# bottledspace/refraction-raytracing-dxr

Hardware: AMD Instinct MI355X
Metric: Mrays/s (primary+refracted) at 1920x1080, monkey.obj (higher is better)
Workload: dtype f32

## Files before the change

refraction_raytracing_dxr_amd/_build.py:

```python
import os
import shutil
import subprocess

PKG = os.path.dirname(os.path.abspath(__file__))
CSRC = os.path.join(PKG, "csrc")
LIB = os.path.join(PKG, "librrdxr.so")
DEMO = os.path.join(PKG, "rrdemo")

DEVICE_SOURCES = ["rr_bvh_build.hip", "rr_render_fused.hip", "rr_render_paths.hip", "rr_render_lds.hip", "rr_render_stream.hip",
                  "rr_query.hip", "rr_query_multi.hip", "rr_frame.hip", "rr_shade_rays.hip", "rr_render_samples.hip",
                  "rr_render_adaptive.hip", "rr_render_lens.hip", "rr_render_spectral.hip", "rr_render_materials.hip"]
HOST_SOURCES = ["rr_capi.cpp", "rr_capi_build.cpp", "rr_capi_dispatch.cpp", "rr_capi_orbit.cpp", "rr_capi_query.cpp", "rr_capi_comm.cpp",
                "rr_choice.cpp", "host/rr_host_camera.cpp", "host/rr_host_mesh.cpp", "host/rr_host_image.cpp", "host/rr_host_partition.cpp",
                "host/Mesh.cpp", "host/RefractionDemo.cpp"]
HEADERS = ["rr_types.h", "rr_context.h", "rr_choice.h", "rr_device.h", "rr_launch.h", "rr_render_common.h", "rr_render_materials.h", "host/Mesh.hpp", "host/RefractionDemo.hpp", "host/rr_host_lens.h",
           "../../include/rrdxr.h"]

COMMON = ["-O3", "-std=c++17", "-fPIC", "-ffp-contract=off", "-fno-fast-math", "-Wall", "-Wno-unused-function"]
DEVICE_FLAGS = ["--offload-arch=gfx950", "-fno-gpu-rdc"] + os.environ.get("RR_EXTRA_DEFINES", "").split()


def _hipcc():
    exe = shutil.which("hipcc") or "/opt/rocm/bin/hipcc"
    if not os.path.exists(exe):
        raise RuntimeError("hipcc not found: the HIP extension cannot be built")
    return exe


def _stale(target, deps):
    if not os.path.exists(target):
        return True
    t = os.path.getmtime(target)
    return any((not os.path.exists(d)) or os.path.getmtime(d) > t for d in deps)


def build(force=False, verbose=False):
    hipcc = _hipcc()
    srcs = [os.path.join(CSRC, s) for s in DEVICE_SOURCES + HOST_SOURCES]
    deps = srcs + [os.path.join(CSRC, h) for h in HEADERS] + [os.path.abspath(__file__)]
    objdir = os.path.join(PKG, "build")
    os.makedirs(objdir, exist_ok=True)
    stamp = os.path.join(objdir, "flags.txt")
# ... 30 lines not shown
```

refraction_raytracing_dxr_amd/csrc/rr_capi.cpp:

```cpp
#include "rr_context.h"

#include <dlfcn.h>
#include <new>

static_assert(CHOICE_TILE == (uint32_t)TILE && CHOICE_STREAM_MAX_GEN == STREAM_MAX_GEN, "rr_choice.h mirrors rr_types.h");

static_assert(sizeof(rr_vertex) == 32, "Vertex stride (Mesh.cpp:45)");
static_assert(sizeof(rr_instance_desc) == 64, "D3D12_RAYTRACING_INSTANCE_DESC");
static_assert(sizeof(rr_scene_constants) == 80, "SceneConstants");
static_assert(sizeof(rr_ray) == sizeof(rr_ray_dev) && sizeof(rr_hit) == sizeof(rr_hit_dev), "ray/hit ABI");
static_assert(offsetof(rr_ray, instance_mask) == 36 && offsetof(rr_ray_dev, instance_mask) == 36, "rr_ray.instance_mask");

namespace {
struct Roctx {
    int (*push)(const char*) = nullptr;
    int (*pop)() = nullptr;
    Roctx()
    {
        for (const char* lib : { "librocprofiler-sdk-roctx.so", "libroctx64.so" }) {
            if (void* h = dlopen(lib, RTLD_LAZY | RTLD_LOCAL)) {
                push = reinterpret_cast<int (*)(const char*)>(dlsym(h, "roctxRangePushA"));
                pop = reinterpret_cast<int (*)()>(dlsym(h, "roctxRangePop"));
                if (push && pop) return;
                push = nullptr; pop = nullptr;
// ... 117 lines not shown
    rr_context* ctx = new (std::nothrow) rr_context();
    if (!ctx) return RR_ERR_OUT_OF_MEMORY;
    ctx->device = device_ordinal;
    ctx->n_cus = prop.multiProcessorCount > 0 ? prop.multiProcessorCount : 256;
    if (hipSetDevice(device_ordinal) != hipSuccess || ctx->own_stream.create(hipStreamNonBlocking) != hipSuccess ||
        ctx->d_cnt.alloc(1) != hipSuccess || ctx->d_tickets.alloc((rr_context::MAX_LANES + 1) * LDS_TICKET_WORDS) != hipSuccess) {
        delete ctx;
        return RR_ERR_DEVICE;
    }
    ctx->stream = ctx->own_stream.get();
    (void)hipMemsetAsync(ctx->d_cnt.get(), 0, sizeof(CounterBlock), ctx->stream);
    (void)hipMemsetAsync(ctx->d_tickets.get(), 0, (rr_context::MAX_LANES + 1) * LDS_TICKET_WORDS * sizeof(uint32_t), ctx->stream);
    if (const char* e = getenv("RR_DEBUG_KERNEL"))
        ctx->dbg.kernel = !strcmp(e, "fused") ? 1 : !strcmp(e, "lds") ? 4 : !strcmp(e, "paths") ? 5 : !strcmp(e, "stream") ? 10 : 0;
    if (const char* e = getenv("RR_DEBUG_STACK")) ctx->dbg.stack = atoi(e);
    if (const char* e = getenv("RR_DEBUG_TICKET")) ctx->dbg_ticket_blocks = atoi(e);
    if (const char* e = getenv("RR_DEBUG_SHAPE")) ctx->dbg_shape = atoi(e);
    if (const char* e = getenv("RR_DEBUG_REFINE_GROUPS")) ctx->dbg_refine_groups = std::max(atoi(e), 0);
    if (const char* e = getenv("RR_DEBUG_TLAS32")) ctx->dbg.tlas32 = atoi(e) != 0;
    if (const char* e = getenv("RR_DEBUG_TILE_ORDER")) ctx->dbg_tile_order = atoi(e) != 0;
    if (const char* e = getenv("RR_DEBUG_ASYNC")) { unsigned l = 2, sh = 2; if (sscanf(e, "%u,%u", &l, &sh) == 2 && l >= 1 && sh >= 1) { ctx->dbg_async[0] = l; ctx->dbg_async[1] = sh; ctx->dbg_async_set = true; } }
    if (const char* e = getenv("RR_DEBUG_DIAG")) ctx->dbg_diag = e;
    if (const char* e = getenv("RR_DEBUG_GROUP_TRACE")) ctx->dbg_group_trace = atoi(e) != 0;
    *out = ctx;
    return RR_OK;
}

int rr_destroy(rr_context* ctx)
{
    if (!ctx) return RR_ERR_INVALID_ARGUMENT;
    (void)hipSetDevice(ctx->device);
    (void)hipStreamSynchronize(ctx->stream);
    for (const Stream& s : ctx->lane_stream) if (s.get()) (void)hipStreamSynchronize(s.get());
    delete ctx;
    return RR_OK;
}

const char* rr_last_error(const rr_context* ctx) { return ctx ? ctx->err.c_str() : "null context"; }

int rr_set_stream(rr_context* ctx, void* hip_stream)
{
    if (int r = use_device(ctx)) return r;
    RR_HIP(hipStreamSynchronize(ctx->stream));
    ctx->stream = (hipStream_t)hip_stream;
    return RR_OK;
}

int rr_reset_stream(rr_context* ctx)
{
    if (int r = use_device(ctx)) return r;
    RR_HIP(hipStreamSynchronize(ctx->stream));
    ctx->stream = ctx->own_stream.get();
    return RR_OK;
}

int rr_wait(rr_context* ctx)
{
    if (int r = use_device(ctx)) return r;
    if (int r = join_lanes(ctx)) return r;
    RR_HIP(hipStreamSynchronize(ctx->stream));
    return RR_OK;
}

int rr_set_frames_in_flight(rr_context* ctx, uint32_t n)
{
    if (int r = use_device(ctx)) return r;
// ... 223 lines not shown
```

refraction_raytracing_dxr_amd/csrc/rr_capi_dispatch.cpp:

```cpp
#include "rr_context.h"

namespace {
int ensure_cams(rr_context* ctx, size_t n)
{
    return n <= ctx->d_cams.size() ? RR_OK : ctx->d_cams.grow(ctx, n < 64 ? 64 : n);
}

constexpr size_t STREAM_BUDGET_MAX = (size_t)48 << 30, STREAM_BUDGET_MIN = (size_t)1 << 30;
constexpr uint32_t STREAM_BLK = 1024;

size_t stream_budget(rr_context* ctx)
{
    if (ctx->strm_budget == 0) {
        size_t free_b = 0, total_b = 0;
        size_t b = STREAM_BUDGET_MAX;
        if (hipMemGetInfo(&free_b, &total_b) == hipSuccess) b = std::min(b, free_b / 6u);
        if (const char* e = getenv("RR_DEBUG_STREAM_BUDGET_GB")) { const long g = atol(e); if (g > 0 && g <= 200) b = (size_t)g << 30; }
        ctx->strm_budget = std::max(b, STREAM_BUDGET_MIN);
    }
    return ctx->strm_budget;
}

uint32_t lds_node_bytes(const MeshRes& m) { return m.n_nodes() * (uint32_t)sizeof(QNode); }

// ... 172 lines not shown
struct Launch {
    SceneDev sc;
    DispatchDev a;
    uint32_t need;
    const rr_scene_constants* h_cams; const rr_dispatch_params* p;
    FusedVariant fused;
};

int ensure_lds_park(rr_context* ctx, uint32_t slot, int max_reflect)
{
    const size_t park_need = (size_t)ctx->n_cus * 32 * (max_reflect <= 2 ? 2u : 8u) * 8 * 64;
    return ctx->d_park[slot].size() < park_need ? ctx->d_park[slot].grow(ctx, park_need) : RR_OK;
}

int launch_lds(rr_context* ctx, const Launch& L, bool stats)
{
    const MeshRes& m0 = ctx->meshes[(size_t)ctx->inst_host[0].blas];
    LdsDispatch q;
    memset(&q, 0, sizeof q);
    const uint32_t slot = stream_slot(ctx);
    q.tickets = ctx->d_tickets.get() + (size_t)slot * LDS_TICKET_WORDS;
    q.park_slots = L.p->max_reflect <= 2 ? 2u : 8u;
    if (int r = ensure_lds_park(ctx, slot, L.p->max_reflect)) return r;
    q.park = ctx->d_park[slot].get();
    uint32_t rect[4];
    (void)rr_host_screen_rect(m0.bounds, ((ctx->dbg_ticket_blocks & 3) == 1 || (L.p->flags & RR_DISPATCH_DEBUG_NO_CULL)) ? nullptr : L.h_cams, L.a.n_frames,
                     L.a.W, L.a.H, rect);
    if ((ctx->dbg_ticket_blocks & 3) == 2) rect[2] = rect[0];
    q.n_queues = (ctx->dbg_ticket_blocks & 64) ? 64u : (ctx->dbg_ticket_blocks & 128) ? LDS_QUEUES : 8u;
    q.home_xcc = (ctx->dbg_ticket_blocks & 16) ? 0u : 1u;
    q.rx0 = rect[0]; q.ry0 = rect[1]; q.rx1 = rect[2]; q.ry1 = rect[3];
    q.node_bytes = lds_node_bytes(m0);
    q.stack_entries = L.need + 1;
    RR_HIP(launch_render_lds(L.sc, L.a, q, ctx->n_cus, stats, ctx->stream, ctx->dbg_shape));
    return RR_OK;
}

int launch_kernel(rr_context* ctx, const Launch& L, int kernel, bool stats)
{
    if (kernel == K_STREAM) return render_stream(ctx, L.sc, L.a, L.a.n_frames, (int)L.need, stats);
    if (kernel == K_LDS) return launch_lds(ctx, L, stats);
    if (kernel == K_PATHS) RR_HIP(launch_render_paths(L.sc, L.a, (int)L.need, stats, ctx->stream));
    else RR_HIP(launch_render_fused(L.sc, L.a, L.fused.stack, L.fused.pend, stats, ctx->stream, L.fused.stack16));
    return RR_OK;
}

int time_candidates(rr_context* ctx, Launch L, int cand_a, int cand_b, float ms[2])
{
    if (cand_b == K_STREAM) if (int r = ensure_stream_buffers(ctx, stream_plan(ctx, L.a, L.a.n_frames))) return r;
    if (cand_a == K_LDS || cand_b == K_LDS) if (int r = ensure_lds_park(ctx, stream_slot(ctx), L.p->max_reflect)) return r;
    for (Event& e : ctx->ch_ev) if (!e.get()) RR_HIP(e.create(hipEventDefault));
    if (!ctx->d_cnt_trial.get()) RR_HIP(ctx->d_cnt_trial.alloc(1));
    RR_HIP(hipDeviceSynchronize());
    RR_HIP(hipMemsetAsync(ctx->d_cnt_trial.get(), 0, sizeof(CounterBlock), ctx->stream));
    point_counters(L.a, ctx->d_cnt_trial.get());
    if (int r = launch_kernel(ctx, L, cand_a, false)) return r;
    for (int c = 0; c < 2; ++c) {
        RR_HIP(hipEventRecord(ctx->ch_ev[2 * c].get(), ctx->stream));
        if (int r = launch_kernel(ctx, L, c == 0 ? cand_a : cand_b, false)) return r;
        RR_HIP(hipEventRecord(ctx->ch_ev[2 * c + 1].get(), ctx->stream));
    }
    RR_HIP(hipEventSynchronize(ctx->ch_ev[3].get()));
    RR_HIP(hipEventElapsedTime(&ms[0], ctx->ch_ev[0].get(), ctx->ch_ev[1].get()));
    RR_HIP(hipEventElapsedTime(&ms[1], ctx->ch_ev[2].get(), ctx->ch_ev[3].get()));
    return RR_OK;
}

// ... 213 lines not shown
```

refraction_raytracing_dxr_amd/csrc/rr_context.h:

```cpp
#pragma once
#include "../../include/rrdxr.h"

#include <hip/hip_runtime.h>

#include <algorithm>
#include <cmath>
#include <cstdio>
#include <cstdlib>
#include <cstring>
#include <string>
#include <vector>

#include "rr_choice.h"
#include "rr_launch.h"

namespace rr {

struct Range {
    explicit Range(const char* name);
    ~Range();
};

template <class T, bool Pinned = false> class Buf {
public:
// ... 121 lines not shown
    bool cam_set = false;
    DevBuf<CamDev> d_cams;
    static constexpr int CAM_SLOTS = 4;
    HostBuf<CamDev> h_cams[CAM_SLOTS];
    Event      h_cams_ev[CAM_SLOTS];
    bool       h_cams_busy[CAM_SLOTS] = {};
    uint32_t   h_cams_next = 0;

    uint32_t tile_rank = 0, tile_world = 1;

    static constexpr uint32_t MAX_LANES = 4;
    Stream      lane_stream[MAX_LANES];
    Event       lane_fork[MAX_LANES], lane_done[MAX_LANES];
    DevBuf<CamDev> lane_cams[MAX_LANES];
    bool        lane_busy[MAX_LANES] = {};
    uint32_t    frames_in_flight = 2;
    size_t      frame_base = 0;

    uint32_t W = 0, H = 0, frame_world = 0, frame_depth = 1;
    DevBuf<uint32_t> d_rgba8;
    DevBuf<float4>   d_f32;
    DevBuf<uint32_t> d_assembled;
    bool      have_f32 = false, have_frame = false, have_assembled = false;
    uint64_t  last_pixels = 0;
    uint64_t  accum_pixels = 0;
    bool      last_stats = false;

    DevBuf<CounterBlock> d_cnt;
    DevBuf<CounterBlock> d_cnt_trial;
    DevBuf<uint32_t> d_park[MAX_LANES + 1];
    char       last_kernel_name[96] = "";
    uint32_t   last_kernel = 0;
    DevBuf<uint32_t> d_tickets;

    DebugFacts dbg = { 0, 0, false };
    int  dbg_ticket_blocks = 0;
    bool dbg_group_trace = true;
    bool dbg_async_set = false;
    uint32_t dbg_async[2] = { 2, 2 };
    bool dbg_tile_order = true;
    int  dbg_shape = 0;
    int  dbg_refine_groups = 0;
    std::string dbg_diag;

    Event ev_begin, ev_end;
    std::vector<Event> kev;
    uint32_t kev_used = 0;

    StreamSet strm[MAX_LANES + 1];
    size_t    strm_budget = 0;
    ChoiceClass ch[3];
    Event      ch_ev[4];

    DevBuf<rr_ray_dev> d_rays;
    DevBuf<rr_hit_dev> d_hits;
    DevBuf<uint32_t>   d_counts;
    DevBuf<float4>     d_out_f32;
    DevBuf<uint32_t>   d_out_rgba8, d_out_n;
    DevBuf<uint32_t>   d_adaptive_taken;
    DevBuf<float4>     d_adaptive_ws;
    DevBuf<MatDev>     d_mats;
    uint32_t n_mats = 0, max_material = 0;
};

namespace rr {

// ... 53 lines not shown
```

refraction_raytracing_dxr_amd/csrc/rr_launch.h:

```cpp
#pragma once
#include <hip/hip_runtime.h>
#include "rr_types.h"
#include "host/rr_host_lens.h"

namespace rr {

struct alignas(16) rr_ray_dev { float origin[3]; float tmin; float dir[3]; float tmax; uint32_t flags; uint32_t instance_mask; uint32_t pad[2]; };
struct rr_hit_dev { float t, u, v; uint32_t prim, inst, hit; };
static_assert(sizeof(rr_ray_dev) == 48 && sizeof(rr_hit_dev) == 24, "ABI layout");

hipError_t launch_render_fused(const SceneDev& sc, const DispatchDev& a, int stack, int pend, bool stats, hipStream_t s,
                               bool stack16 = false);
const char* last_render_kernel_name();
void set_render_kernel_name(const char* fmt, ...) __attribute__((format(printf, 1, 2)));
hipError_t launch_render_paths(const SceneDev& sc, const DispatchDev& a, int stack, bool stats, hipStream_t s);
int lds_kernel_shape(uint32_t node_bytes, uint32_t stack_entries, size_t* lds_bytes, int min_shape = 0);
hipError_t launch_render_lds(const SceneDev& sc, const DispatchDev& a, LdsDispatch q, int n_cus, bool stats, hipStream_t s, int min_shape = 0);
hipError_t launch_render_stream(const SceneDev& sc, const DispatchDev& a, const StreamDev& s, int stack, uint32_t n_wg, bool stats, hipStream_t st);
hipError_t launch_env_lookup(const SceneDev& sc, const float* dirs, uint32_t n, float* rgb, hipStream_t s);
hipError_t launch_trace_rays(const SceneDev& sc, const rr_ray_dev* rays, uint32_t n, rr_hit_dev* hits, uint32_t* err,
                             int stack, hipStream_t s);
hipError_t launch_query_rays(const SceneDev& sc, const rr_ray_dev* rays, uint32_t n, rr_hit_dev* hits, uint32_t inst0_mask, int stack,
                             hipStream_t s);
constexpr uint32_t RR_QUERY_MULTI_MAX_K = 16;
hipError_t launch_query_multi(const SceneDev& sc, const rr_ray_dev* rays, uint32_t n, uint32_t k, rr_hit_dev* hits, uint32_t* counts,
                              uint32_t inst0_mask, int stack, hipStream_t s);
hipError_t launch_shade_rays(const SceneDev& sc, const DispatchDev& a, const rr_ray_dev* rays, uint32_t n, float4* f32, uint32_t* rgba8,
                             uint32_t* n_rays, int stack, int pend, bool stack16, hipStream_t s);
struct SampleOffsets { static constexpr uint32_t MAX = 64; float v[2 * MAX]; };
hipError_t launch_render_samples(const SceneDev& sc, const DispatchDev& a, const CamDev& cam, const SampleOffsets& off, uint32_t n_samples,
                                 float4* f32, uint32_t* rgba8, uint32_t* n_rays, int stack, int pend, bool stack16, hipStream_t s);
hipError_t launch_render_lens(const SceneDev& sc, const DispatchDev& a, const CamDev& cam, const SampleOffsets& off, const SampleOffsets& loff,
                              const LensDev& lens, uint32_t n_samples, float4* f32, uint32_t* rgba8, uint32_t* n_rays, int stack, int pend,
                              bool stack16, hipStream_t s);
struct BandTable { static constexpr uint32_t MAX = SampleOffsets::MAX; float ior[MAX]; float inv_ior[MAX]; float weight[MAX][3]; };
hipError_t launch_render_spectral(const SceneDev& sc, const DispatchDev& a, const CamDev& cam, const SampleOffsets& off, const BandTable& bands,
                                  uint32_t n_samples, float4* f32, uint32_t* rgba8, uint32_t* n_rays, int stack, int pend, bool stack16,
                                  hipStream_t s);
hipError_t launch_shade_rays_mat(const SceneDev& sc, const DispatchDev& a, const MatDev* mats, uint32_t mat0, const rr_ray_dev* rays, uint32_t n,
                                 float4* f32, uint32_t* rgba8, uint32_t* n_rays, int stack, int pend, bool stack16, hipStream_t s);
hipError_t launch_render_materials(const SceneDev& sc, const DispatchDev& a, const CamDev& cam, const SampleOffsets& off, const MatDev* mats,
                                   uint32_t mat0, uint32_t n_samples, float4* f32, uint32_t* rgba8, uint32_t* n_rays, int stack, int pend,
                                   bool stack16, hipStream_t s);
struct AdaptiveWorkspace {
    float4* rec; uint32_t* cnt; uint32_t* list; unsigned long long* masks; uint32_t* base; uint32_t* total;
    uint64_t bytes;
    AdaptiveWorkspace(void* p, uint32_t W, uint32_t H)
    {
        const uint64_t n = (uint64_t)W * H, nb = (uint64_t)((W + 7u) / 8u) * ((H + 7u) / 8u);
        const uint64_t o_cnt = 16u * n, o_list = o_cnt + 4u * n, o_masks = (o_list + 4u * n + 15u) & ~(uint64_t)15u, o_base = o_masks + 8u * nb;
// ... 57 lines not shown
```

refraction_raytracing_dxr_amd/csrc/rr_render_common.h:

```cpp
#pragma once
#include <hip/hip_runtime.h>
#include <type_traits>
#include "rr_device.h"
#include "rr_launch.h"

#ifndef RR_FUSED_WAVES_PER_SIMD
#define RR_FUSED_WAVES_PER_SIMD(STACK) ((STACK) <= 19 ? 8 : (STACK) <= 22 ? 7 : (STACK) <= 26 ? 6 : (STACK) <= 31 ? 5 : (STACK) <= 39 ? 4 : 2)
#endif
#ifndef RR_TLAS_WAVES_PER_SIMD
#define RR_TLAS_WAVES_PER_SIMD(STACK) ((STACK) <= 31 ? 5 : (STACK) <= 39 ? 4 : 2)
#endif

namespace rr {


struct PendRay {
    float ox, oy, oz, dx, dy, dz, w;
    uint32_t meta;
};

__device__ __forceinline__ uint32_t compact1by1(uint32_t v)
{
    v &= 0x55555555u;
    v = (v ^ (v >> 1)) & 0x33333333u;
// ... 230 lines not shown
        p3[0] = (uint8_t)packed; p3[1] = (uint8_t)(packed >> 8); p3[2] = (uint8_t)(packed >> 16);
    } else {
        out_rgba8[o] = packed;
    }
    if (out_f32) out_f32[o] = make_float4(acc.x, acc.y, acc.z, 1.0f);
}

template <bool STATS>
__device__ __forceinline__ void flush_stats(const DispatchDev& a, const LaneStats& st, uint32_t shard, uint32_t lane)
{
    uint32_t wr = wave_reduce_add(st.rays);
    if (lane == 0 && wr) atomicAdd(&a.ray_shards[shard & (RAY_SHARDS - 1)], wr);
    if (STATS) {
        uint32_t v;
        v = wave_reduce_add(st.hits);  if (lane == 0 && v) atomicAdd(&a.counters[C_HITS], (unsigned long long)v);
        v = wave_reduce_add(st.miss);  if (lane == 0 && v) atomicAdd(&a.counters[C_MISSES], (unsigned long long)v);
        v = wave_reduce_add(st.term);  if (lane == 0 && v) atomicAdd(&a.counters[C_TERMINAL], (unsigned long long)v);
        v = wave_reduce_add(st.tir);   if (lane == 0 && v) atomicAdd(&a.counters[C_TIR], (unsigned long long)v);
        v = wave_reduce_add(st.cnt.nodes); if (lane == 0 && v) atomicAdd(&a.counters[C_NODES], (unsigned long long)v);
        v = wave_reduce_add(st.cnt.tris);  if (lane == 0 && v) atomicAdd(&a.counters[C_TRIS], (unsigned long long)v);
        v = wave_reduce_add(st.pixels); if (lane == 0 && v) atomicAdd(&a.counters[C_PRIMARY], (unsigned long long)v);
        v = wave_reduce_add(st.cnt.node_trips); if (lane == 0 && v) atomicAdd(&a.counters[C_NODE_TRIPS], (unsigned long long)v);
        v = wave_reduce_add(st.cnt.leaf_trips); if (lane == 0 && v) atomicAdd(&a.counters[C_LEAF_TRIPS], (unsigned long long)v);
        v = wave_reduce_add(st.passes); if (lane == 0 && v) atomicAdd(&a.counters[C_PASSES], (unsigned long long)v);
        if (lane == 0 && st.blocks) atomicAdd(&a.counters[C_WAVES], (unsigned long long)st.blocks);
        if (lane == 0 && st.bg_blocks) atomicAdd(&a.counters[C_BG_WAVES], (unsigned long long)st.bg_blocks);
        if (lane == 0 && (st.blocks || st.rays)) {
            atomicAdd(&a.counters[C_CLK_TICKS], (unsigned long long)(__builtin_amdgcn_s_memtime() - st.clk0));
            atomicAdd(&a.counters[C_CLK_REAL], (unsigned long long)(__builtin_amdgcn_s_memrealtime() - st.rt0));
        }
    }
}

__device__ __forceinline__ uint32_t tile_in_launch_order(const DispatchDev& a, uint32_t i, uint32_t limit)
{
    if (a.rt_w == 0u || i >= limit) return i;
    const uint32_t n_rect = a.rt_w * a.rt_h;
    if (i < n_rect) {
        const uint32_t row = a.rt_w == 1u ? i : __umulhi(i, a.rt_div_w);
        return (a.rt_y0 + row) * a.tiles_x + a.rt_x0 + (i - row * a.rt_w);
    }
    uint32_t j = i - n_rect;
    const uint32_t above = a.rt_y0 * a.tiles_x;
    if (j < above) return j;
    j -= above;
    const uint32_t per_row = a.tiles_x - a.rt_w, beside = per_row * a.rt_h;
    if (j < beside) {
        const uint32_t row = per_row == 1u ? j : __umulhi(j, a.rt_div_o), c = j - row * per_row;
        return (a.rt_y0 + row) * a.tiles_x + (c < a.rt_x0 ? c : c + a.rt_w);
    }
    return (a.rt_y0 + a.rt_h) * a.tiles_x + (j - beside);
}

struct BlockPos { uint32_t frame, tile_local, x0, y0, px0, py0; bool tile_ok, bg; };
__device__ __forceinline__ BlockPos wave_block_pos(const DispatchDev& a, uint32_t wb)
{
    BlockPos p;
    const uint32_t blk = wb >> 2, wave = wb & 3u;
    p.frame = blk % a.n_frames;
    uint32_t strip;
    block_to_tile(blk / a.n_frames, p.tile_local, strip);
    p.tile_ok = p.tile_local < a.n_local_tiles;
    p.bg = false;
    uint32_t tile;
    if (a.mesh_part) {
        const uint32_t k = p.tile_local;
// ... 16 lines not shown
```

refraction_raytracing_dxr_amd/csrc/rr_render_lds.hip:

```cpp
#include <hip/hip_runtime.h>
#include "rr_render_common.h"

namespace rr {

__device__ __forceinline__ BlockPos lds_tile_block(const DispatchDev& a, const LdsDispatch& q, uint32_t u, uint32_t j)
{
    BlockPos p;
    const uint32_t tile = a.n_frames == 1u ? u : __umulhi(u, q.div_frames);
    p.frame = u - tile * a.n_frames;
    p.tile_local = tile;
    p.tile_ok = tile < a.n_local_tiles;
    p.bg = false;
    const uint32_t ty = a.tiles_x == 1u ? tile : __umulhi(tile, q.div_tiles_x), tx = tile - ty * a.tiles_x;
    p.px0 = (j & 3u) * 8u; p.py0 = (j >> 2) * 8u;
    p.x0 = tx * TILE + p.px0; p.y0 = ty * TILE + p.py0;
    return p;
}

__device__ __forceinline__ BlockPos lds_rect_block(const DispatchDev& a, const LdsDispatch& q, uint32_t u, uint32_t j)
{
    BlockPos p;
    const uint32_t strip = a.n_frames == 1u ? u : __umulhi(u, q.div_frames), per_row = q.rect_bw >> 2;
    p.frame = u - strip * a.n_frames;
    const uint32_t row = per_row == 1u ? strip : __umulhi(strip, q.div_per_row), col = strip - row * per_row;
// ... 132 lines not shown
        if (w_arrived + 1u == (uint32_t)NW) {
            const uint32_t arrived = atomicAdd(&q.tickets[2u * LDS_QUEUES * 16u], 1u);
            if (arrived + 1u == gridDim.x) {
                for (uint32_t k = 0; k <= 2u * LDS_QUEUES; ++k) atomicExch(&q.tickets[k * 16u], 0u);
            }
        }
    }
}

constexpr struct { int nw, wgs; } LDS_SHAPES[] = { { 12, 2 }, { 16, 2 }, { 16, 1 } };
static size_t lds_shape_bytes(int i, uint32_t node_bytes, uint32_t stack_entries) { return (size_t)node_bytes + (size_t)LDS_SHAPES[i].nw * stack_entries * 64 * sizeof(uint16_t); }

int lds_kernel_shape(uint32_t node_bytes, uint32_t stack_entries, size_t* lds_bytes, int min_shape)
{
    for (int i = min_shape < 0 ? 0 : min_shape; i < 3; ++i) {
        const size_t need = lds_shape_bytes(i, node_bytes, stack_entries);
        if (need <= (size_t)(160 * 1024) / LDS_SHAPES[i].wgs - 512) { if (lds_bytes) *lds_bytes = need; return i; }
        if (min_shape <= 0) break;
    }
    return -1;
}

template <int SHAPE, bool STATS, bool DIAG = false>
static hipError_t launch_lds_nw(const SceneDev& sc, const DispatchDev& a, const LdsDispatch& q, int n_cus, hipStream_t s)
{
    constexpr int NW = LDS_SHAPES[SHAPE].nw, WGS = LDS_SHAPES[SHAPE].wgs;
    static const hipError_t attr = hipFuncSetAttribute(reinterpret_cast<const void*>(&k_render_lds<NW, WGS, STATS, DIAG>), hipFuncAttributeMaxDynamicSharedMemorySize, 159 * 1024);
    if (attr != hipSuccess) return attr;
    if (!DIAG) set_render_kernel_name("k_render_lds<%d, %d, %s, false>", NW, WGS, STATS ? "true" : "false");
    hipLaunchKernelGGL((k_render_lds<NW, WGS, STATS, DIAG>), dim3((uint32_t)n_cus * WGS), dim3(NW * 64), lds_shape_bytes(SHAPE, q.node_bytes, q.stack_entries), s, sc, a, q);
    return hipGetLastError();
}

hipError_t launch_render_lds(const SceneDev& sc, const DispatchDev& a, LdsDispatch q, int n_cus, bool stats, hipStream_t s, int min_shape)
{
    if (a.n_blocks == 0) return hipSuccess;
    const int shape = lds_kernel_shape(q.node_bytes, q.stack_entries, nullptr, min_shape);
    if (shape < 0) return hipErrorInvalidValue;
    {
        const uint32_t grid = (uint32_t)n_cus * (uint32_t)LDS_SHAPES[shape].wgs;
        if (q.n_queues > grid) q.n_queues = grid;
        if (q.n_queues > LDS_QUEUES) q.n_queues = LDS_QUEUES;
        if (q.n_queues < 1u) q.n_queues = 1u;
    }
    q.p2_tickets = a.n_local_tiles * a.n_frames;
    if (q.rx1 > q.rx0 && q.ry1 > q.ry0) {
        q.rx0 &= ~31u;
        q.rx1 = (q.rx1 + 31u) & ~31u;
    }
    const bool rect = q.rx1 > q.rx0 && q.ry1 > q.ry0;
    q.rect_bw = rect ? (q.rx1 - q.rx0) / 8u : 0u;
    q.p1_tickets = !rect ? 0u : (q.rect_bw / 4u) * ((q.ry1 - q.ry0) / 8u) * a.n_frames;
    if ((uint64_t)q.p2_tickets * a.n_frames >= 0xffffffffull || (uint64_t)q.p1_tickets * a.n_frames >= 0xffffffffull) return hipErrorInvalidValue;
    q.div_frames = (uint32_t)(0x100000000ull / a.n_frames) + 1u;
    q.div_tiles_x = (uint32_t)(0x100000000ull / a.tiles_x) + 1u;
    q.div_per_row = rect ? (uint32_t)(0x100000000ull / (q.rect_bw / 4u)) + 1u : 0u;
    static_assert(sizeof LDS_SHAPES / sizeof LDS_SHAPES[0] == 3, "lds_kernel_shape and the rungs below");
    if (a.diag) return launch_lds_nw<0, false, true>(sc, a, q, n_cus, s);
    if (shape == 0) return stats ? launch_lds_nw<0, true>(sc, a, q, n_cus, s) : launch_lds_nw<0, false>(sc, a, q, n_cus, s);
    if (shape == 1) return stats ? launch_lds_nw<1, true>(sc, a, q, n_cus, s) : launch_lds_nw<1, false>(sc, a, q, n_cus, s);
    return stats ? launch_lds_nw<2, true>(sc, a, q, n_cus, s) : launch_lds_nw<2, false>(sc, a, q, n_cus, s);
}

}
```

refraction_raytracing_dxr_amd/csrc/rr_render_stream.hip:

```cpp
#include <hip/hip_runtime.h>
#include "rr_render_common.h"

#ifndef RR_STREAM_WPS
#define RR_STREAM_WPS 6
#endif

namespace rr {

constexpr uint32_t SQ_BLK = 1024;
constexpr uint32_t SQ_NONE = 0xffffffffu;
constexpr uint32_t SQ_DEAD = 0xfffffffeu;
constexpr int TRAV_FIN = (int)0x80000001;
constexpr int TRAV_IDLE = (int)0x80000002;
constexpr uint8_t PIX_BLACK = 0, PIX_ONE_LEAF = 1, PIX_LEAVES = 2;

__device__ __forceinline__ void sq_finalize(const StreamDev& s, uint32_t qsel, uint32_t base, uint32_t used, uint32_t lane)
{
    if (lane < SQ_BLK / 64u) {
        const uint32_t lo = lane * 64u;
        s.fill[qsel][(base >> 6) + lane] = used > lo ? (used - lo < 64u ? used - lo : 64u) : 0u;
    }
}

__device__ __forceinline__ void sq_push(const StreamDev& s, uint32_t gen_out, uint32_t& base, uint32_t& used, bool have, f3 O, f3 D,
// ... 336 lines not shown
                    const uint32_t rank = __builtin_amdgcn_mbcnt_hi((uint32_t)(need >> 32), __builtin_amdgcn_mbcnt_lo((uint32_t)need, 0u));
                    if (node == TRAV_IDLE && rank < left) {
                        const uint32_t r = chunk * 64u + off + rank;
                        const uint32_t m = __float_as_uint(qin[(size_t)r * 3 + 2].x);
                        const float4 q0 = qin[(size_t)r * 3], q1 = qin[(size_t)r * 3 + 1];
                        rid = r;
                        start_ray(mk3(q0.x, q0.y, q0.z), mk3(q1.x, q1.y, q1.z), (m & META_INSIDE) != 0u, true);
                    }
                    const uint32_t asked = (uint32_t)__popcll(need);
                    off += asked < left ? asked : left;
                    need = __ballot(node == TRAV_IDLE);
                }
            }
        }
    }
    if (MODE != 2 && ob != SQ_NONE && ob != SQ_DEAD) sq_finalize(s, (gen + 1u) & 1u, ob, ou, lane);
    flush_stats<STATS>(a, st, blockIdx.x * 4u + wave, lane);
}

template <bool STATS>
__global__ __launch_bounds__(256) void k_stream_background(SceneDev sc, DispatchDev a, StreamDev s)
{
    const uint32_t wave = __builtin_amdgcn_readfirstlane(threadIdx.x >> 6), lane = threadIdx.x & 63u;
    const uint32_t wb = s.n_rect_wb + blockIdx.x * 4u + wave;
    LaneStats st;
    stats_clock_begin<STATS>(st);
    if (wb < a.n_blocks * 4u) {
        const BlockPos bp = wave_block_pos(a, wb);
        const uint32_t lx = compact1by1(lane), ly = compact1by1(lane >> 1);
        const uint32_t x = bp.x0 + lx, y = bp.y0 + ly;
        st.blocks = bp.tile_ok ? 1u : 0u;
        if (STATS) st.bg_blocks = st.blocks;
        if (bp.tile_ok && x < a.W && y < a.H) {
            const CamDev& cb = a.cams[bp.frame];
            const f3 D = camera_ray_dir(cb.M, a.sx[x], a.sy[y]);
            st.pixels = 1; st.rays = 1;
            if (STATS) { st.miss = 1; if (first_active_lane()) st.passes = 1; }
            const f3 e = env_lookup(sc, D);
            const f3 acc = mk3(fmaf(1.0f, e.x, 0.0f), fmaf(1.0f, e.y, 0.0f), fmaf(1.0f, e.z, 0.0f));
            const size_t o = a.compact_out == 0u ? (size_t)y * a.W + x : (size_t)bp.tile_local * (TILE * TILE) + (bp.py0 + ly) * TILE + (bp.px0 + lx);
            uint32_t* const out = bp.bg ? a.out_bg + (size_t)bp.frame * a.bg_stride : a.out_rgba8 + (size_t)bp.frame * a.frame_stride;
            store_pixel(a, out, a.out_f32 ? a.out_f32 + (size_t)bp.frame * a.frame_stride : nullptr, o, acc);
        }
    }
    flush_stats<STATS>(a, st, blockIdx.x * 4u + wave, lane);
}

__global__ __launch_bounds__(256) void k_stream_resolve(DispatchDev a, StreamDev s)
{
    const uint32_t wave = __builtin_amdgcn_readfirstlane(threadIdx.x >> 6), lane = threadIdx.x & 63u;
    const uint32_t wb = blockIdx.x * 4u + wave;
    if (wb >= s.n_rect_wb) return;
    const BlockPos bp = wave_block_pos(a, wb);
    const uint32_t lx = compact1by1(lane), ly = compact1by1(lane >> 1);
    const uint32_t x = bp.x0 + lx, y = bp.y0 + ly;
    if (!bp.tile_ok || x >= a.W || y >= a.H) return;
    const uint32_t cov = wb * 64u + lane;
    const uint8_t kind = s.pending[cov];
    const float4* sl = s.slots + (size_t)cov * 4;
    f3 acc = mk3(0.0f, 0.0f, 0.0f);
    if (kind == PIX_ONE_LEAF) {
        const float4 v = sl[0];
        acc = mk3(fmaf(v.x, v.y, 0.0f), fmaf(v.x, v.z, 0.0f), fmaf(v.x, v.w, 0.0f));
    } else if (kind == PIX_LEAVES) {
#pragma unroll
        for (int k = 0; k < 4; ++k) {
            const float4 v = sl[k];
            acc.x = fmaf(v.x, v.y, acc.x); acc.y = fmaf(v.x, v.z, acc.y); acc.z = fmaf(v.x, v.w, acc.z);
        }
    }
    const size_t o = a.compact_out == 0u ? (size_t)y * a.W + x : (size_t)bp.tile_local * (TILE * TILE) + (bp.py0 + ly) * TILE + (bp.px0 + lx);
    uint32_t* const out = bp.bg ? a.out_bg + (size_t)bp.frame * a.bg_stride : a.out_rgba8 + (size_t)bp.frame * a.frame_stride;
    store_pixel(a, out, a.out_f32 ? a.out_f32 + (size_t)bp.frame * a.frame_stride : nullptr, o, acc);
}

// ... 37 lines not shown
```

refraction_raytracing_dxr_amd/csrc/rr_types.h:

```cpp
#pragma once
#include <math.h>
#include <stdint.h>

namespace rr {

struct alignas(16) BvhNode {
    float lox[2], loy[2];
    float loz[2], hix[2];
    float hiy[2], hiz[2];
    int32_t c[2];
    uint32_t pad[2];
};
static_assert(sizeof(BvhNode) == 64, "BvhNode must be 64 B");

struct QGrid { float org[3]; float cell[3]; };
struct alignas(16) QNode {
    uint32_t lox, loy, loz, hix;
    uint32_t hiy, hiz;
    int32_t c[2];
};
static_assert(sizeof(QNode) == 32, "QNode must be 32 B");

struct alignas(16) TriRec {
    float v0[3]; uint32_t prim;
// ... 103 lines not shown
    const float k = floorf(fmaf(x, 1.44269504f, 0.5f));
    float r = fmaf(k, -0.693359375f, x);
    r = fmaf(k, 2.12194440e-4f, r);
    float p = 1.9875691500e-4f;
    p = fmaf(p, r, 1.3981999507e-3f);
    p = fmaf(p, r, 8.3334519073e-3f);
    p = fmaf(p, r, 4.1665795894e-2f);
    p = fmaf(p, r, 1.6666665459e-1f);
    p = fmaf(p, r, 5.0000001201e-1f);
    const float y = fmaf(p, r * r, r) + 1.0f;
    const uint32_t two_k = (uint32_t)((int32_t)k + 127) << 23;
    return y * __builtin_bit_cast(float, two_k);
}

struct LdsDispatch {
    uint32_t* tickets;
    uint32_t p1_tickets;
    uint32_t pad0;
    uint32_t rect_bw;
    uint32_t rx0, ry0, rx1, ry1;
    uint32_t p2_tickets;
    uint32_t pad1, pad2;
    uint32_t n_queues;
    uint32_t home_xcc;
    uint32_t* park;
    uint32_t park_slots;
    uint32_t node_bytes;
    uint32_t stack_entries;
    uint32_t div_frames, div_tiles_x, div_per_row;
};
constexpr uint32_t LDS_QUEUES = 512;
constexpr uint32_t LDS_TICKET_WORDS = (2 * LDS_QUEUES + 1) * 16;

struct MeshPartDev { uint32_t tiles_x, n_tiles, rect_x0, rect_y0, rect_w, rect_h, world, rounds; };
#if defined(__HIPCC__)
__device__ __forceinline__ void mesh_deal_owner(uint32_t i, uint32_t world, uint32_t j, uint32_t& rank, uint32_t& slot)
{
    if (j == 0u || world == 1u) { rank = i % world; slot = i / world; return; }
    if (j == 0xffffffffu) { rank = 1u + i % (world - 1u); slot = i / (world - 1u); return; }
    const uint32_t cl = j * (world - 1u) + 1u, c = i / cl, pos = i % cl;
    if (pos == cl - 1u) { rank = 0u; slot = c; }
    else { rank = 1u + pos % (world - 1u); slot = c * j + pos / (world - 1u); }
}
__device__ __forceinline__ uint32_t mesh_deal_index(uint32_t rank, uint32_t k, uint32_t world, uint32_t j)
{
    if (j == 0u || world == 1u) return k * world + rank;
    if (j == 0xffffffffu) return k * (world - 1u) + (rank - 1u);
    const uint32_t cl = j * (world - 1u) + 1u;
    if (rank == 0u) return k * cl + cl - 1u;
    return (k / j) * cl + (k % j) * (world - 1u) + (rank - 1u);
}
#endif

constexpr uint32_t STREAM_MAX_GEN = 64;
struct StreamDev {
    float4*   q[2];
    uint32_t* fill[2];
    uint32_t* heads;
    uint32_t* next;
    float4*   slots;
    uint8_t*  pending;
    uint32_t  cap;
    uint32_t  n_rect_wb;
};

enum Counter : int {
// ... 11 lines not shown
```

Baseline: 32050.

## Render background tiles in a separate kernel on a forked stream

Result: slower. 31180 (-2.7%).

```diff
diff --git a/refraction_raytracing_dxr_amd/_build.py b/refraction_raytracing_dxr_amd/_build.py
--- a/refraction_raytracing_dxr_amd/_build.py
+++ b/refraction_raytracing_dxr_amd/_build.py
@@ -7,7 +7,7 @@
 LIB = os.path.join(PKG, "librrdxr.so")
 DEMO = os.path.join(PKG, "rrdemo")
 
-DEVICE_SOURCES = ["rr_bvh_build.hip", "rr_render_fused.hip", "rr_render_paths.hip", "rr_render_lds.hip", "rr_render_stream.hip",
+DEVICE_SOURCES = ["rr_bvh_build.hip", "rr_render_fused.hip", "rr_render_paths.hip", "rr_render_lds.hip", "rr_render_background.hip", "rr_render_stream.hip",
                   "rr_query.hip", "rr_query_multi.hip", "rr_frame.hip", "rr_shade_rays.hip", "rr_render_samples.hip",
                   "rr_render_adaptive.hip", "rr_render_lens.hip", "rr_render_spectral.hip", "rr_render_materials.hip"]
 HOST_SOURCES = ["rr_capi.cpp", "rr_capi_build.cpp", "rr_capi_dispatch.cpp", "rr_capi_orbit.cpp", "rr_capi_query.cpp", "rr_capi_comm.cpp",
diff --git a/refraction_raytracing_dxr_amd/csrc/rr_capi.cpp b/refraction_raytracing_dxr_amd/csrc/rr_capi.cpp
--- a/refraction_raytracing_dxr_amd/csrc/rr_capi.cpp
+++ b/refraction_raytracing_dxr_amd/csrc/rr_capi.cpp
@@ -173,6 +173,7 @@
     (void)hipSetDevice(ctx->device);
     (void)hipStreamSynchronize(ctx->stream);
     for (const Stream& s : ctx->lane_stream) if (s.get()) (void)hipStreamSynchronize(s.get());
+    for (const Stream& s : ctx->bg_stream) if (s.get()) (void)hipStreamSynchronize(s.get());
     delete ctx;
     return RR_OK;
 }
diff --git a/refraction_raytracing_dxr_amd/csrc/rr_capi_dispatch.cpp b/refraction_raytracing_dxr_amd/csrc/rr_capi_dispatch.cpp
--- a/refraction_raytracing_dxr_amd/csrc/rr_capi_dispatch.cpp
+++ b/refraction_raytracing_dxr_amd/csrc/rr_capi_dispatch.cpp
@@ -228,7 +228,25 @@
     q.rx0 = rect[0]; q.ry0 = rect[1]; q.rx1 = rect[2]; q.ry1 = rect[3];
     q.node_bytes = lds_node_bytes(m0);
     q.stack_entries = L.need + 1;
-    RR_HIP(launch_render_lds(L.sc, L.a, q, ctx->n_cus, stats, ctx->stream, ctx->dbg_shape));
+    lds_widen_rect(q);
+    LdsBackground g;
+    const bool apart = !(ctx->dbg_ticket_blocks & 256) && L.a.n_blocks != 0 && lds_background_plan(L.a, q, &g);
+    const bool second = apart && g.n_tiles != 0;
+    if (second) {
+        if (!ctx->bg_stream[slot].get()) {
+            RR_HIP(ctx->bg_stream[slot].create(hipStreamNonBlocking));
+            RR_HIP(ctx->bg_fork[slot].create(hipEventDisableTiming));
+            RR_HIP(ctx->bg_join[slot].create(hipEventDisableTiming));
+        }
+        RR_HIP(hipEventRecord(ctx->bg_fork[slot].get(), ctx->stream));
+    }
+    RR_HIP(launch_render_lds(L.sc, L.a, q, ctx->n_cus, stats, ctx->stream, ctx->dbg_shape, apart));
+    if (second) {
+        RR_HIP(hipStreamWaitEvent(ctx->bg_stream[slot].get(), ctx->bg_fork[slot].get(), 0));
+        RR_HIP(launch_lds_background(L.sc, L.a, g, stats, ctx->bg_stream[slot].get()));
+        RR_HIP(hipEventRecord(ctx->bg_join[slot].get(), ctx->bg_stream[slot].get()));
+        RR_HIP(hipStreamWaitEvent(ctx->stream, ctx->bg_join[slot].get(), 0));
+    }
     return RR_OK;
 }
 
diff --git a/refraction_raytracing_dxr_amd/csrc/rr_context.h b/refraction_raytracing_dxr_amd/csrc/rr_context.h
--- a/refraction_raytracing_dxr_amd/csrc/rr_context.h
+++ b/refraction_raytracing_dxr_amd/csrc/rr_context.h
@@ -177,6 +177,8 @@
     char       last_kernel_name[96] = "";
     uint32_t   last_kernel = 0;
     DevBuf<uint32_t> d_tickets;
+    Stream     bg_stream[MAX_LANES + 1];
+    Event      bg_fork[MAX_LANES + 1], bg_join[MAX_LANES + 1];
 
     DebugFacts dbg = { 0, 0, false };
     int  dbg_ticket_blocks = 0;
diff --git a/refraction_raytracing_dxr_amd/csrc/rr_launch.h b/refraction_raytracing_dxr_amd/csrc/rr_launch.h
--- a/refraction_raytracing_dxr_amd/csrc/rr_launch.h
+++ b/refraction_raytracing_dxr_amd/csrc/rr_launch.h
@@ -15,7 +15,11 @@
 void set_render_kernel_name(const char* fmt, ...) __attribute__((format(printf, 1, 2)));
 hipError_t launch_render_paths(const SceneDev& sc, const DispatchDev& a, int stack, bool stats, hipStream_t s);
 int lds_kernel_shape(uint32_t node_bytes, uint32_t stack_entries, size_t* lds_bytes, int min_shape = 0);
-hipError_t launch_render_lds(const SceneDev& sc, const DispatchDev& a, LdsDispatch q, int n_cus, bool stats, hipStream_t s, int min_shape = 0);
+hipError_t launch_render_lds(const SceneDev& sc, const DispatchDev& a, LdsDispatch q, int n_cus, bool stats, hipStream_t s, int min_shape = 0,
+                             bool background_apart = false);
+void lds_widen_rect(LdsDispatch& q);
+bool lds_background_plan(const DispatchDev& a, const LdsDispatch& q, LdsBackground* g);
+hipError_t launch_lds_background(const SceneDev& sc, const DispatchDev& a, const LdsBackground& g, bool stats, hipStream_t s);
 hipError_t launch_render_stream(const SceneDev& sc, const DispatchDev& a, const StreamDev& s, int stack, uint32_t n_wg, bool stats, hipStream_t st);
 hipError_t launch_env_lookup(const SceneDev& sc, const float* dirs, uint32_t n, float* rgb, hipStream_t s);
 hipError_t launch_trace_rays(const SceneDev& sc, const rr_ray_dev* rays, uint32_t n, rr_hit_dev* hits, uint32_t* err,
diff --git a/refraction_raytracing_dxr_amd/csrc/rr_render_background.hip b/refraction_raytracing_dxr_amd/csrc/rr_render_background.hip
--- /dev/null
+++ b/refraction_raytracing_dxr_amd/csrc/rr_render_background.hip
@@ -0,0 +1,99 @@
+#include <hip/hip_runtime.h>
+#include "rr_render_common.h"
+
+namespace rr {
+
+__device__ __forceinline__ uint32_t background_tile(const DispatchDev& a, const LdsBackground& g, uint32_t i)
+{
+    const uint32_t above = g.in_y0 * a.tiles_x;
+    if (i < above) return i;
+    const uint32_t j = i - above, per_row = a.tiles_x - g.in_w, beside = per_row * g.in_h;
+    if (j < beside) {
+        const uint32_t row = per_row == 1u ? j : __umulhi(j, g.div_beside), c = j - row * per_row;
+        return (g.in_y0 + row) * a.tiles_x + (c < g.in_x0 ? c : c + g.in_w);
+    }
+    return (g.in_y0 + g.in_h) * a.tiles_x + (j - beside);
+}
+
+__device__ __forceinline__ bool background_block(const SceneDev& sc, const DispatchDev& a, const LdsBackground& g, uint32_t b, uint32_t wave,
+                                                 uint32_t lane, LaneStats& st)
+{
+    const uint32_t s = a.n_frames == 1u ? b : __umulhi(b, g.div_frames), frame = b - s * a.n_frames;
+    const uint32_t i = s >> 2, py0 = (s & 3u) * 8u, px0 = wave * 8u;
+    if (i >= g.n_tiles) return false;
+    const uint32_t tile = background_tile(a, g, i);
+    const uint32_t ty = a.tiles_x == 1u ? tile : __umulhi(tile, g.div_tiles_x), tx = tile - ty * a.tiles_x;
+    const uint32_t x0 = tx * TILE + px0, y0 = ty * TILE + py0;
+    if (x0 >= g.rx0 && x0 < g.rx1 && y0 >= g.ry0 && y0 < g.ry1) return false;
+    const uint32_t lx = compact1by1(lane), ly = compact1by1(lane >> 1);
+    const uint32_t x = x0 + lx, y = y0 + ly;
+    if (x < a.W && y < a.H) {
+        const size_t o = a.compact_out == 0u ? (size_t)y * a.W + x : (size_t)tile * (TILE * TILE) + (py0 + ly) * TILE + (px0 + lx);
+        background_pixel<false>(sc, a, a.cams[frame], x, y, a.out_rgba8 + (size_t)frame * a.frame_stride,
+                                a.out_f32 ? a.out_f32 + (size_t)frame * a.frame_stride : nullptr, o, st);
+    }
+    return true;
+}
+
+constexpr uint32_t LDS_BG_STATS_GROUPS = 2048;
+template <bool STATS>
+__global__ __launch_bounds__(256) void k_lds_background(SceneDev sc, DispatchDev a, LdsBackground g, uint32_t n_slots)
+{
+    const uint32_t wave = __builtin_amdgcn_readfirstlane(threadIdx.x >> 6), lane = threadIdx.x & 63u;
+    const uint32_t shard = blockIdx.x * 4u + wave;
+    if (STATS) {
+        LaneStats st;
+        stats_clock_begin<true>(st);
+        uint32_t n_blocks = 0u, n_pixels = 0u, n_passes = 0u;
+#pragma unroll 1
+        for (uint32_t b = blockIdx.x; b < n_slots; b += gridDim.x) {
+            LaneStats one;
+            if (!background_block(sc, a, g, b, wave, lane, one)) continue;
+            const uint32_t n = (uint32_t)__popcll(__ballot(one.rays != 0u));
+            n_blocks += 1u; n_pixels += n; n_passes += n != 0u ? 1u : 0u;
+        }
+        st.blocks = st.bg_blocks = n_blocks;
+        st.pixels = st.rays = st.miss = lane == 0 ? n_pixels : 0u;
+        st.passes = lane == 0 ? n_passes : 0u;
+        flush_stats<true>(a, st, shard, lane);
+        return;
+    }
+    LaneStats st;
+    (void)background_block(sc, a, g, blockIdx.x, wave, lane, st);
+    const uint32_t wr = (uint32_t)__popcll(__ballot(st.rays != 0u));
+    if (lane == 0 && wr) atomicAdd(&a.ray_shards[shard & (RAY_SHARDS - 1)], wr);
+}
+
+bool lds_background_plan(const DispatchDev& a, const LdsDispatch& q, LdsBackground* g)
+{
+    if (a.tile_world != 1u || a.n_local_tiles != a.n_tiles || a.tiles_x == 0u || a.n_frames == 0u || a.diag) return false;
+    const bool seen = a.hx1 > a.hx0 && a.hy1 > a.hy0;
+    if (seen && !(a.hx0 >= q.rx0 && a.hx1 <= q.rx1 && a.hy0 >= q.ry0 && a.hy1 <= q.ry1)) return false;
+    *g = LdsBackground{};
+    g->rx0 = q.rx0; g->ry0 = q.ry0; g->rx1 = q.rx1; g->ry1 = q.ry1;
+    const uint32_t tiles_y = a.n_tiles / a.tiles_x;
+    if (q.rx1 > q.rx0 && q.ry1 > q.ry0) {
+        const uint32_t x0 = (q.rx0 + TILE - 1u) / TILE, x1 = q.rx1 / TILE < a.tiles_x ? q.rx1 / TILE : a.tiles_x;
+        const uint32_t y0 = (q.ry0 + TILE - 1u) / TILE, y1 = q.ry1 / TILE < tiles_y ? q.ry1 / TILE : tiles_y;
+        if (x1 > x0 && y1 > y0) { g->in_x0 = x0; g->in_y0 = y0; g->in_w = x1 - x0; g->in_h = y1 - y0; }
+    }
+    g->n_tiles = a.n_tiles - g->in_w * g->in_h;
+    const uint64_t grid = (uint64_t)g->n_tiles * 4u * a.n_frames;
+    if (grid * a.n_frames >= 0xffffffffull || grid > 0x7fffffffull) return false;
+    g->div_frames = (uint32_t)(0x100000000ull / a.n_frames) + 1u;
+    g->div_tiles_x = (uint32_t)(0x100000000ull / a.tiles_x) + 1u;
+    g->div_beside = a.tiles_x > g->in_w ? (uint32_t)(0x100000000ull / (a.tiles_x - g->in_w)) + 1u : 0u;
+    return true;
+}
+
+hipError_t launch_lds_background(const SceneDev& sc, const DispatchDev& a, const LdsBackground& g, bool stats, hipStream_t s)
+{
+    const uint64_t grid = (uint64_t)g.n_tiles * 4u * a.n_frames;
+    if (grid == 0u) return hipSuccess;
+    const uint32_t n_slots = (uint32_t)grid;
+    if (stats) hipLaunchKernelGGL((k_lds_background<true>), dim3(n_slots < LDS_BG_STATS_GROUPS ? n_slots : LDS_BG_STATS_GROUPS), dim3(256), 0, s, sc, a, g, n_slots);
+    else hipLaunchKernelGGL((k_lds_background<false>), dim3(n_slots), dim3(256), 0, s, sc, a, g, n_slots);
+    return hipGetLastError();
+}
+
+}
diff --git a/refraction_raytracing_dxr_amd/csrc/rr_render_common.h b/refraction_raytracing_dxr_amd/csrc/rr_render_common.h
--- a/refraction_raytracing_dxr_amd/csrc/rr_render_common.h
+++ b/refraction_raytracing_dxr_amd/csrc/rr_render_common.h
@@ -286,6 +286,18 @@
     }
 }
 
+template <bool STATS>
+__device__ __forceinline__ void background_pixel(const SceneDev& sc, const DispatchDev& a, const CamDev& cb, uint32_t x, uint32_t y,
+                                                 uint32_t* out_rgba8, float4* out_f32, size_t o, LaneStats& st)
+{
+    const f3 D = camera_ray_dir(cb.M, a.sx[x], a.sy[y]);
+    st.pixels += 1; st.rays += 1;
+    if (STATS) { st.miss += 1; if (first_active_lane()) st.passes += 1; }
+    const f3 e = env_lookup(sc, D);
+    const f3 acc = mk3(fmaf(1.0f, e.x, 0.0f), fmaf(1.0f, e.y, 0.0f), fmaf(1.0f, e.z, 0.0f));
+    store_pixel(a, out_rgba8, out_f32, o, acc);
+}
+
 __device__ __forceinline__ uint32_t tile_in_launch_order(const DispatchDev& a, uint32_t i, uint32_t limit)
 {
     if (a.rt_w == 0u || i >= limit) return i;
diff --git a/refraction_raytracing_dxr_amd/csrc/rr_render_lds.hip b/refraction_raytracing_dxr_amd/csrc/rr_render_lds.hip
--- a/refraction_raytracing_dxr_amd/csrc/rr_render_lds.hip
+++ b/refraction_raytracing_dxr_amd/csrc/rr_render_lds.hip
@@ -188,7 +188,15 @@
     return hipGetLastError();
 }
 
-hipError_t launch_render_lds(const SceneDev& sc, const DispatchDev& a, LdsDispatch q, int n_cus, bool stats, hipStream_t s, int min_shape)
+void lds_widen_rect(LdsDispatch& q)
+{
+    if (q.rx1 > q.rx0 && q.ry1 > q.ry0) {
+        q.rx0 &= ~31u;
+        q.rx1 = (q.rx1 + 31u) & ~31u;
+    }
+}
+
+hipError_t launch_render_lds(const SceneDev& sc, const DispatchDev& a, LdsDispatch q, int n_cus, bool stats, hipStream_t s, int min_shape, bool background_apart)
 {
     if (a.n_blocks == 0) return hipSuccess;
     const int shape = lds_kernel_shape(q.node_bytes, q.stack_entries, nullptr, min_shape);
@@ -200,14 +208,12 @@
         if (q.n_queues < 1u) q.n_queues = 1u;
     }
     q.p2_tickets = a.n_local_tiles * a.n_frames;
-    if (q.rx1 > q.rx0 && q.ry1 > q.ry0) {
-        q.rx0 &= ~31u;
-        q.rx1 = (q.rx1 + 31u) & ~31u;
-    }
+    lds_widen_rect(q);
     const bool rect = q.rx1 > q.rx0 && q.ry1 > q.ry0;
     q.rect_bw = rect ? (q.rx1 - q.rx0) / 8u : 0u;
     q.p1_tickets = !rect ? 0u : (q.rect_bw / 4u) * ((q.ry1 - q.ry0) / 8u) * a.n_frames;
     if ((uint64_t)q.p2_tickets * a.n_frames >= 0xffffffffull || (uint64_t)q.p1_tickets * a.n_frames >= 0xffffffffull) return hipErrorInvalidValue;
+    if (background_apart && !a.diag) q.p2_tickets = 0u;
     q.div_frames = (uint32_t)(0x100000000ull / a.n_frames) + 1u;
     q.div_tiles_x = (uint32_t)(0x100000000ull / a.tiles_x) + 1u;
     q.div_per_row = rect ? (uint32_t)(0x100000000ull / (q.rect_bw / 4u)) + 1u : 0u;
diff --git a/refraction_raytracing_dxr_amd/csrc/rr_render_stream.hip b/refraction_raytracing_dxr_amd/csrc/rr_render_stream.hip
--- a/refraction_raytracing_dxr_amd/csrc/rr_render_stream.hip
+++ b/refraction_raytracing_dxr_amd/csrc/rr_render_stream.hip
@@ -392,15 +392,9 @@
         st.blocks = bp.tile_ok ? 1u : 0u;
         if (STATS) st.bg_blocks = st.blocks;
         if (bp.tile_ok && x < a.W && y < a.H) {
-            const CamDev& cb = a.cams[bp.frame];
-            const f3 D = camera_ray_dir(cb.M, a.sx[x], a.sy[y]);
-            st.pixels = 1; st.rays = 1;
-            if (STATS) { st.miss = 1; if (first_active_lane()) st.passes = 1; }
-            const f3 e = env_lookup(sc, D);
-            const f3 acc = mk3(fmaf(1.0f, e.x, 0.0f), fmaf(1.0f, e.y, 0.0f), fmaf(1.0f, e.z, 0.0f));
             const size_t o = a.compact_out == 0u ? (size_t)y * a.W + x : (size_t)bp.tile_local * (TILE * TILE) + (bp.py0 + ly) * TILE + (bp.px0 + lx);
             uint32_t* const out = bp.bg ? a.out_bg + (size_t)bp.frame * a.bg_stride : a.out_rgba8 + (size_t)bp.frame * a.frame_stride;
-            store_pixel(a, out, a.out_f32 ? a.out_f32 + (size_t)bp.frame * a.frame_stride : nullptr, o, acc);
+            background_pixel<STATS>(sc, a, a.cams[bp.frame], x, y, out, a.out_f32 ? a.out_f32 + (size_t)bp.frame * a.frame_stride : nullptr, o, st);
         }
     }
     flush_stats<STATS>(a, st, blockIdx.x * 4u + wave, lane);
diff --git a/refraction_raytracing_dxr_amd/csrc/rr_types.h b/refraction_raytracing_dxr_amd/csrc/rr_types.h
--- a/refraction_raytracing_dxr_amd/csrc/rr_types.h
+++ b/refraction_raytracing_dxr_amd/csrc/rr_types.h
@@ -159,6 +159,13 @@
 constexpr uint32_t LDS_QUEUES = 512;
 constexpr uint32_t LDS_TICKET_WORDS = (2 * LDS_QUEUES + 1) * 16;
 
+struct LdsBackground {
+    uint32_t rx0, ry0, rx1, ry1;
+    uint32_t in_x0, in_y0, in_w, in_h;
+    uint32_t n_tiles;
+    uint32_t div_frames, div_tiles_x, div_beside;
+};
+
 struct MeshPartDev { uint32_t tiles_x, n_tiles, rect_x0, rect_y0, rect_w, rect_h, world, rounds; };
 #if defined(__HIPCC__)
 __device__ __forceinline__ void mesh_deal_owner(uint32_t i, uint32_t world, uint32_t j, uint32_t& rank, uint32_t& slot)
```
